# danyang-rainbow/trlx-t5

Measured on AMD Instinct MI355X. Metric: PPO experience+loss tokens/sec and % HBM roofline, 1/2/4/8 MI355X, higher is better.
Workload: dtype f32; 1 GPU; C2 GPT-2 sentiments PPO shape: 128 x 48 response tokens, vocab 50257, bf16 logits; rows_per_gpu=128, global_batch=128, seq_len=48, vocab=50257, logits_dtype=bf16, parallelism=dp1, schedule=pipelined

## Files before the change

include/trlx_t5_amd.h:

```cpp
#ifndef TRLX_T5_AMD_H
#define TRLX_T5_AMD_H

#include <stdint.h>

#ifdef __cplusplus
extern "C" {
#endif

#define TRLX_ABI_VERSION 2

typedef enum {
    TRLX_F32 = 0,
    TRLX_BF16 = 1,
    TRLX_I64 = 2,
} trlx_dtype;

typedef enum {
    TRLX_OK = 0,
    TRLX_ERR_SHAPE = 1,
    TRLX_ERR_STRIDE = 2,
    TRLX_ERR_DTYPE = 3,
    TRLX_ERR_LAUNCH = 4,
    TRLX_ERR_ARG = 5,
} trlx_status;
// ... 506 lines not shown
    float* rew_kl;
    float* rew_score;
    double* stats8;
    int mom_lag;
    void* workspace;
} trlx_gae_split_args;
int trlx_ppo_loss_rows_split_gae(const void* logits, int dtype, int64_t B, int64_t T, int64_t V, int64_t sb,
                                 int64_t st, const int64_t* labels, int64_t lb, int64_t lt, const void* old_lp,
                                 int old_dtype, const float* adv0, const float* adv_kl, const float* rew_kl,
                                 const float* rew_score, const double* stats8, int unbiased, const double* ctl_state,
                                 float kl_coef, float* coef, const double* msum, const int64_t* mask,
                                 const void* values, int v_dtype, const void* old_values, int ov_dtype,
                                 float* rewards, void* returns, int r_dtype, float cliprange, float cliprange_value,
                                 float vf_coef, float* lp_out, void* dx, int64_t dsb, int64_t dst, float* dvalues,
                                 void* workspace, const trlx_gae_split_args* gae, void* stream, void* done_event);

int trlx_comm_load(const char* librccl_path);
int64_t trlx_comm_unique_id_bytes(void);
int trlx_comm_unique_id(void* id_out, int64_t nbytes);
int trlx_comm_init(void** comm_out, const void* id, int64_t nbytes, int nranks, int rank);
int trlx_comm_allreduce_sum_f64(void* comm, double* buf, int64_t n, void* stream);
int trlx_comm_destroy(void* comm);

int trlx_scale_by(const void* x, void* out, int dtype, int64_t n, const float* scale, void* stream);

#ifdef __cplusplus
}
#endif
#endif
```

trlx-t5_amd/_lib.py:

```python
import contextlib
import ctypes
import os

import torch

_HERE = os.path.dirname(os.path.abspath(__file__))
LIB_PATH = os.environ.get("TRLX_T5_AMD_LIB") or os.path.join(_HERE, "libtrlx_t5_amd.so")

F32, BF16, I64 = 0, 1, 2
ABI_VERSION = 2
MOMENT_SLOTS = 4
SPLIT_MOMENT_SLOTS = 8
PPO_STATS = 13
PPO_PARTIAL_SLOTS = 16

_c_vp, _c_i64, _c_int, _c_f, _c_d = ctypes.c_void_p, ctypes.c_int64, ctypes.c_int, ctypes.c_float, ctypes.c_double


class IlqlArgs(ctypes.Structure):
    _fields_ = [
        ("dtype", _c_int), ("nq", _c_int),
        ("B", _c_i64), ("L", _c_i64), ("A", _c_i64), ("V", _c_i64),
        ("logits", _c_vp), ("logits_sb", _c_i64), ("logits_st", _c_i64),
        ("q", _c_vp * 2), ("q_sb", _c_i64 * 2), ("q_st", _c_i64 * 2),
# ... 236 lines not shown
    "trlx_ppo_rollout_loss_ctl": (_c_int, [_c_i64, _c_i64, _c_vp, _c_f, _c_vp, _c_vp, _c_vp, _kl_ctl_p, _c_vp]),
    "trlx_ppo_rollout_gae_split": (_c_int, [_c_i64, _c_i64, _c_vp, _c_vp, _c_vp, _c_int, _c_vp, _c_vp, _c_vp,
                                            _score_ctl_p, _c_f, _c_d, _c_d, _c_vp, _c_vp, _c_vp, _c_vp, _c_vp,
                                            _c_vp, _c_vp, _c_int, _c_int, _c_vp, _c_vp, _c_vp]),
    "trlx_score_moments_merge": (_c_int, [_c_vp, _c_vp, _c_vp, _c_vp]),
    "trlx_ppo_whiten_coef": (_c_int, [_c_vp, _c_int, _c_vp, _c_f, _c_vp, _c_vp]),
    "trlx_ppo_loss_rows_split": (_c_int, [_c_vp, _c_int, _c_i64, _c_i64, _c_i64, _c_i64, _c_i64, _c_vp, _c_i64,
                                          _c_i64, _c_vp, _c_int, _c_vp, _c_vp, _c_vp, _c_vp, _c_vp, _c_vp, _c_vp,
                                          _c_vp, _c_int, _c_vp, _c_int, _c_vp, _c_vp, _c_int, _c_f, _c_f, _c_f,
                                          _c_vp, _c_vp, _c_i64, _c_i64, _c_vp, _c_vp, _c_vp]),
    "trlx_ppo_loss_rows_split_gae": (_c_int, [_c_vp, _c_int, _c_i64, _c_i64, _c_i64, _c_i64, _c_i64, _c_vp, _c_i64,
                                              _c_i64, _c_vp, _c_int, _c_vp, _c_vp, _c_vp, _c_vp, _c_vp, _c_int, _c_vp,
                                              _c_f, _c_vp, _c_vp, _c_vp, _c_vp, _c_int, _c_vp, _c_int, _c_vp, _c_vp,
                                              _c_int, _c_f, _c_f, _c_f, _c_vp, _c_vp, _c_i64, _c_i64, _c_vp, _c_vp,
                                              _gae_split_p, _c_vp, _c_vp]),
    "trlx_comm_load": (_c_int, [ctypes.c_char_p]),
    "trlx_comm_unique_id_bytes": (_c_i64, []),
    "trlx_comm_unique_id": (_c_int, [_c_vp, _c_i64]),
    "trlx_comm_init": (_c_int, [ctypes.POINTER(ctypes.c_void_p), _c_vp, _c_i64, _c_int, _c_int]),
    "trlx_comm_allreduce_sum_f64": (_c_int, [_c_vp, _c_vp, _c_i64, _c_vp]),
    "trlx_comm_destroy": (_c_int, [_c_vp]),
    "trlx_lsm_gather_fwd_loss_tail": (_c_int, [_c_vp, _c_vp, _c_int, _c_i64, _c_i64, _c_i64, _c_i64, _c_i64, _c_vp,
                                               _c_i64, _c_i64, _c_vp, _c_vp, _c_vp, _c_vp, _c_int, _c_i64, _c_i64,
                                               _c_vp, _c_f, _c_vp, _c_vp, _c_vp, _kl_ctl_p, _c_vp]),
    "trlx_ilql_workspace_bytes": (_c_i64, [_c_i64, _c_i64, _c_i64, _c_int]),
    "trlx_ilql_prep": (_c_int, [_ilql_p, _c_vp]),
    "trlx_ilql_rows": (_c_int, [_ilql_p, _c_vp]),
    "trlx_ilql_finalize": (_c_int, [_ilql_p, _c_vp]),
    "trlx_ilql_loss_fused": (_c_int, [_ilql_p, _c_vp]),
    "trlx_ilql_tq_at_actions": (_c_int, [_ilql_tq_p, _c_vp]),
# ... 43 lines not shown
    _lib = lib
    return lib


def call(name, *args):
    lib = load()
    rc = getattr(lib, name)(*args)
    if rc != 0:
        msg = lib.trlx_last_error().decode(errors="replace")
        err = ValueError if rc in (1, 2, 3, 5) else TrlxError
        raise err(f"{name} failed (status {rc}): {msg}")
    return rc


_TUNED = {}


def set_tuning(key: str, value: int):
    call("trlx_set_tuning", key.encode(), int(value))
    _TUNED[key] = int(value)


@contextlib.contextmanager
def tuning(**knobs):
    prev = {k: _TUNED.get(k, 0) for k in knobs}
    try:
        for k, v in knobs.items():
            set_tuning(k, v)
        yield
    finally:
        for k, v in prev.items():
            set_tuning(k, v)


def query(name, *args):
    return getattr(load(), name)(*args)


def dtype_code(t):
    if t.dtype == torch.float32:
# ... 21 lines not shown
```

trlx-t5_amd/csrc/vocab_rows.hip:

```cpp
#include <string>

#include <hip/hip_ext.h>

#include "ppo_token.h"
#include "row_order.h"

namespace trlx {

enum RowMode { kFwd = 0, kBwd = 1, kPpo = 2 };

struct RowArgs {
    const void* x0;
    const void* x1;
    int64_t B, T, V, sb, st;
    const int64_t* labels;
    int64_t lb, lt;
    void* lp0;
    void* lp1;
    int out_dtype;
    float* lse0;
    float* lse1;
    const float* lse_in;
    const void* grad;
    int grad_dtype;
// ... 20 lines not shown
    int lead_blocks;
    void* done_event;
    const float* coef;
    const float* adv_kl;
    const float* rew_kl;
    const float* rew_score;
    float* rewards_out;
    const double* wstats;
    int wunbiased;
    const double* wctl;
    float wbeta;
    float* coef_out;
    const int64_t* lengths;
    const int* row_list;
    int* order_ws;
};

__global__ void k_whiten_coef(const double* stats, int unbiased, const double* ctl_state, float host_beta,
                              float* coef) {
    if (threadIdx.x == 0)
        whiten_coef_split(stats, unbiased, ctl_state ? float(ctl_state[TRLX_CTL_KL_COEF]) : host_beta, coef);
}

__global__ __launch_bounds__(kRolloutThreads) void k_rollout_loss(LossRolloutArgs L) {
    __shared__ double red[kRolloutsPerBlock * 16];
    loss_tail_block(L, int(blockIdx.x), int(gridDim.x), red);
}

template <class DT>
struct Row {
// ... 116 lines not shown

__device__ __forceinline__ bool any_masked(const RowArgs& a) {
    const double msum = a.msum ? *a.msum : a.msum_host;
    return msum != double(a.B * a.T);
}

template <class DT>
__device__ __forceinline__ void masked_row(const RowArgs& a, int64_t row) {
    typedef typename DT::elem_t E;
    const int64_t b = row / a.T, t = row - b * a.T;
    E* drow = reinterpret_cast<E*>(a.dx) + b * a.dsb + t * a.dst;
    const RowSplit<DT> s(drow, a.V);
    const int tid = threadIdx.x, nthr = blockDim.x;
    const __amdgpu_buffer_rsrc_t rout = make_rsrc(drow + s.head, uint32_t(s.nvec) * 16u);
    const vec4u z = {0u, 0u, 0u, 0u};
    for (int i = tid; i < int(s.nvec); i += nthr) store_grad_b128(z, rout, i * 16, a.spol);
    if (tid < s.head) DT::store1(drow, tid, 0.0f);
    if (tid < s.tail) DT::store1(drow, s.tail0 + tid, 0.0f);
    if (tid == 0) {
        float vin[3];
        const PpoScalars p = ppo_scalars(a, row, vin, true);
        PolicyTerms pt;
        ppo_policy_dlp(0.0f, p.olp, p.A, p.m, p.inv_msum, a.cliprange, pt);
        a.lp_out[row] = 0.0f;
        token_record(a, row, pt, p, vin);
        if (a.coef || a.wstats) split_outputs(a, row, p);
    }
}

template <class DT, int NV, int MODE, bool SAME_PHASE, bool LB512, int NL, int WPE, bool MASKED>
__device__ __forceinline__ void vocab_row(const RowArgs& a, int64_t row) {
    __shared__ float sh_max[kMaxThreads / kWave];
    __shared__ float sh_max2[kMaxThreads / kWave];
// ... 213 lines not shown
                    DT::unpack(lds_row[kk * 512 + tid], f);
#pragma unroll
                    for (int e = 0; e < EPV; ++e) {
                        const int64_t j = r.s.head + int64_t(i) * EPV + e;
                        DT::store1(drow, j, j == r.y ? gy : ng * exp2_fast(fmaf(f[e], kLog2e, lse_l2e)));
                    }
                }
            }
        }
    }
    if (MODE == kPpo && tid == 0) {
        const PolicyTerms t2 = {s_tok[0], s_tok[1], s_tok[2], s_tok[3] != 0.f};
        const PpoScalars p2 = {0.f, s_tok[4], s_tok[5], 0.f, s_ps[7], s_ps[8], s_ps[9], s_ps[10], s_ps[11]};
        token_record(a, r.row, t2, p2, s_ps + 4);
        if (a.coef || a.wstats) split_outputs(a, r.row, p2);
    }
}

template <class DT, int NV, int MODE, bool SAME_PHASE, bool LB512, int NL = 0, int WPE = 4, bool MASKED = false>
__global__ __launch_bounds__((LB512 || NL) ? 512 : kMaxThreads, LB512 ? 8 : (NL ? WPE : 1)) void k_vocab_rows(RowArgs a) {
    if constexpr (MODE == kFwd) {
        if (int(blockIdx.x) < a.tail_blocks) {
            __shared__ double tail_red[kMaxThreads / kWave * 16];
            if (blockIdx.y == 0) loss_tail_block(a.tail, int(blockIdx.x), a.tail_blocks, tail_red);
            return;
        }
    }
    if constexpr (MODE == kPpo && NL > 0) {
        if (int(blockIdx.x) < a.gae_blocks) {
            __shared__ double gae_red[kMaxThreads / kWave * 8];
// ... 147 lines not shown
                    DT::store1(drow, j, j == r.y ? gy : f[e]);
                }
            }
        }
    }
    if (je >= 0) DT::store1(drow, je, je == r.y ? gy : ng * exp2_fast(fmaf(ex, kLog2e, lse_l2e)));
    if (MODE == kPpo && a.tokrec && tid == 0) {
        PpoScalars p2 = ps;
        if (a.coef || a.wstats)
            split_value_inputs(a, r.row, split_advantage(a, r.row, ps.beta), vin, p2.R);
        else
            loss_token_inputs(a.ltok, r.row, vin);
        token_record(a, r.row, pt, ps, vin);
        if (a.coef || a.wstats) split_outputs(a, r.row, p2);
    }
}

struct Geometry {
    int nv;
    int threads;
};

static TuneKnob g_row_variant{0};
static TuneKnob g_resident_threads{0};
static TuneKnob g_resident_lb512{0};
static TuneKnob g_stream_threads{0};
static TuneKnob g_stream_unroll{0};
static TuneKnob g_row_order{0};
static TuneKnob g_ragged_order{0};
static TuneKnob g_order_launch{0};
static TuneKnob g_store_pol{0};
constexpr double kSC1Bytes = 1.5e9;

static int store_policy_for(double grad_bytes, bool split) {
    if (g_store_pol == 5) return kStoreNT;
    if (g_store_pol) return g_store_pol;
    return (!split && grad_bytes > kSC1Bytes) ? kStoreSC1 : kStoreNT;
}
static TuneKnob g_split_lds{0};
static TuneKnob g_split_mid{0};
int tuning_split_lds() { return g_split_lds; }
static TuneKnob g_ilql_split{0};
int tuning_ilql_split() { return g_ilql_split; }

static const int kNVs[] = {1, 2, 3, 4, 5, 6, 7, 8, 10, 12, 13, 16};

// ... 58 lines not shown

static int rows_grid(RowArgs& a, int threads, int nten, hipStream_t stream, dim3& grid, bool split) {
    const int rc = lead_standalone(a, stream, false, !split || threads < kRolloutThreads);
    if (rc) return rc;
    a.tail_blocks = a.has_tail ? int((a.tail.B + threads / kWave - 1) / (threads / kWave)) : 0;
    a.gae_blocks = a.has_gae ? int((a.gae.B + kRolloutsPerBlock - 1) / kRolloutsPerBlock) : 0;
    a.lead_blocks = a.tail_blocks + a.gae_blocks;
    grid = dim3(unsigned(a.B * a.T + a.lead_blocks), unsigned(nten));
    return TRLX_OK;
}

template <int MODE, class DT>
static int launch_rows_dt(const RowArgs& a0, int nten, hipStream_t stream) {
    RowArgs a = a0;
    a.order = g_row_order;
    const double grad_bytes = double(a.B) * double(a.T) * double(a.V) * double(sizeof(typename DT::elem_t));
    a.spol = MODE == kFwd ? kStoreNT : store_policy_for(grad_bytes, true);
    if constexpr (sizeof(typename DT::elem_t) == 2) {
        const int64_t nvec = a.V / 8 + 1 + (kLineVecs - 1);
        const bool want = g_split_lds == 2 || (g_split_lds == 0 && MODE != kFwd);
        if (want && !g_row_variant && !g_resident_threads && nvec > 512 * 8 && nvec <= 512 * (9 + 4)) {
            dim3 grid;
            const int rc = rows_grid(a, 512, nten, stream, grid, true);
            if (rc) return rc;
            if (MODE == kFwd || rows_same_phase(a, 2))
                TRLX_RESIDENT_LAUNCH(DT, 9, true, false, 4, 6, grid, dim3(512), stream, a);
            else
                TRLX_RESIDENT_LAUNCH(DT, 9, false, false, 4, 6, grid, dim3(512), stream, a);
            return check_launch("k_vocab_rows (split LDS, bf16)");
        }
// ... 335 lines not shown
                                         int64_t lb, int64_t lt, const void* values, int v_dtype,
                                         const float* scores, const int64_t* lengths, const int64_t* mask,
                                         float kl_coef, double gamma, double lam, float* lp, float* ref_lp,
                                         float* rewards, float* adv_raw, void* ret, int ret_dtype,
                                         double* stats, void* workspace, void* stream) {
    TRLX_REQUIRE(ref_logits && workspace, TRLX_ERR_ARG, "NULL reference logits / workspace");
    Workspace ws;
    carve_workspace(workspace, B, T, &ws);
    int rc = trlx_lsm_gather_fwd_ragged(logits, ref_logits, dtype, B, T, V, sb, st, labels, lb, lt, lengths, ws.order,
                                        lp, ref_lp, TRLX_F32, stream);
    if (rc) return rc;
    return trlx_ppo_rollout_gae(B, T, lp, ref_lp, values, v_dtype, scores, lengths, mask, kl_coef, gamma, lam,
                                rewards, adv_raw, ret, ret_dtype, stats, workspace, stream);
}

extern "C" int trlx_ppo_loss_rows(const void* logits, int dtype, int64_t B, int64_t T, int64_t V, int64_t sb,
                                  int64_t st, const int64_t* labels, int64_t lb, int64_t lt, const void* old_lp,
                                  int old_dtype, const float* adv_raw, const double* stats, int unbiased,
                                  const int64_t* mask, const void* values, int v_dtype, const void* old_values,
                                  int ov_dtype, const void* returns, int r_dtype, float cliprange,
                                  float cliprange_value, float vf_coef, float* lp_out, void* dx, int64_t dsb,
                                  int64_t dst, float* dvalues, void* workspace, void* stream) {
    RowArgs a = {};
    a.x0 = logits; a.B = B; a.T = T; a.V = V; a.sb = sb; a.st = st; a.labels = labels; a.lb = lb; a.lt = lt;
    a.old_lp = old_lp; a.old_dtype = old_dtype; a.adv = adv_raw; a.stats = stats; a.unbiased = unbiased;
    a.mask = mask; a.msum = stats ? stats + 3 : nullptr; a.msum_host = double(B * T); a.cliprange = cliprange;
    a.lp_out = lp_out; a.dx = dx; a.dsb = dsb; a.dst = dst;
    int rc = check_rows(a, dtype);
    if (rc) return rc;
    TRLX_REQUIRE(B > 0 && T > 0, TRLX_ERR_SHAPE, "empty rollout batch");
    TRLX_REQUIRE(old_lp && adv_raw && stats && values && old_values && returns && lp_out && dx && dvalues && workspace,
                 TRLX_ERR_ARG, "NULL argument to trlx_ppo_loss_rows");
    Workspace ws;
    carve_workspace(workspace, B, T, &ws);
    a.tokrec = ws.tokrec;
    a.ltok.values = values; a.ltok.v_dtype = v_dtype; a.ltok.old_values = old_values; a.ltok.ov_dtype = ov_dtype;
    a.ltok.returns = returns; a.ltok.r_dtype = r_dtype; a.ltok.cv = cliprange_value; a.ltok.vf_coef = vf_coef;
    a.ltok.dv = dvalues;
    return launch_rows<kPpo>(a, dtype, 1, (hipStream_t)stream);
}

extern "C" int trlx_ppo_loss_rows_split(const void* logits, int dtype, int64_t B, int64_t T, int64_t V, int64_t sb,
                                        int64_t st, const int64_t* labels, int64_t lb, int64_t lt, const void* old_lp,
                                        int old_dtype, const float* adv0, const float* adv_kl, const float* rew_kl,
                                        const float* rew_score, const float* coef, const double* msum,
                                        const int64_t* mask, const void* values, int v_dtype, const void* old_values,
                                        int ov_dtype, float* rewards, void* returns, int r_dtype, float cliprange,
                                        float cliprange_value, float vf_coef, float* lp_out, void* dx, int64_t dsb,
                                        int64_t dst, float* dvalues, void* workspace, void* stream) {
    RowArgs a = {};
    a.x0 = logits; a.B = B; a.T = T; a.V = V; a.sb = sb; a.st = st; a.labels = labels; a.lb = lb; a.lt = lt;
    a.old_lp = old_lp; a.old_dtype = old_dtype; a.adv = adv0; a.adv_kl = adv_kl; a.rew_kl = rew_kl;
    a.rew_score = rew_score; a.coef = coef; a.rewards_out = rewards;
    a.mask = mask; a.msum = msum; a.msum_host = double(B * T); a.cliprange = cliprange;
    a.lp_out = lp_out; a.dx = dx; a.dsb = dsb; a.dst = dst;
    int rc = check_rows(a, dtype);
    if (rc) return rc;
    TRLX_REQUIRE(B > 0 && T > 0, TRLX_ERR_SHAPE, "empty rollout batch");
    TRLX_REQUIRE(old_lp && adv0 && adv_kl && rew_kl && rew_score && coef && rewards && values && old_values &&
                 returns && lp_out && dx && dvalues && workspace, TRLX_ERR_ARG,
                 "NULL argument to trlx_ppo_loss_rows_split");
    TRLX_REQUIRE(r_dtype == TRLX_F32 || r_dtype == TRLX_BF16, TRLX_ERR_DTYPE, "returns dtype %d", r_dtype);
    Workspace ws;
    carve_workspace(workspace, B, T, &ws);
    a.tokrec = ws.tokrec;
    a.ltok.values = values; a.ltok.v_dtype = v_dtype; a.ltok.old_values = old_values; a.ltok.ov_dtype = ov_dtype;
    a.ltok.returns = returns; a.ltok.r_dtype = r_dtype; a.ltok.cv = cliprange_value; a.ltok.vf_coef = vf_coef;
    a.ltok.dv = dvalues;
    return launch_rows<kPpo>(a, dtype, 1, (hipStream_t)stream);
}

extern "C" int trlx_ppo_loss_rows_split_gae(
    const void* logits, int dtype, int64_t B, int64_t T, int64_t V, int64_t sb, int64_t st, const int64_t* labels,
    int64_t lb, int64_t lt, const void* old_lp, int old_dtype, const float* adv0, const float* adv_kl,
    const float* rew_kl, const float* rew_score, const double* stats8, int unbiased, const double* ctl_state,
    float kl_coef, float* coef, const double* msum, const int64_t* mask, const void* values, int v_dtype,
    const void* old_values, int ov_dtype, float* rewards, void* returns, int r_dtype, float cliprange,
    float cliprange_value, float vf_coef, float* lp_out, void* dx, int64_t dsb, int64_t dst, float* dvalues,
    void* workspace, const trlx_gae_split_args* gae, void* stream, void* done_event) {
    RowArgs a = {};
    a.x0 = logits; a.B = B; a.T = T; a.V = V; a.sb = sb; a.st = st; a.labels = labels; a.lb = lb; a.lt = lt;
    a.old_lp = old_lp; a.old_dtype = old_dtype; a.adv = adv0; a.adv_kl = adv_kl; a.rew_kl = rew_kl;
    a.rew_score = rew_score; a.rewards_out = rewards;
    a.wstats = stats8; a.wunbiased = unbiased; a.wctl = ctl_state; a.wbeta = kl_coef; a.coef_out = coef;
    a.mask = mask; a.msum = msum; a.msum_host = double(B * T); a.cliprange = cliprange;
    a.lp_out = lp_out; a.dx = dx; a.dsb = dsb; a.dst = dst;
    a.done_event = done_event;
    int rc = check_rows(a, dtype);
    if (rc) return rc;
    TRLX_REQUIRE(B > 0 && T > 0, TRLX_ERR_SHAPE, "empty rollout batch");
    TRLX_REQUIRE(old_lp && adv0 && adv_kl && rew_kl && rew_score && stats8 && rewards && values && old_values &&
                 returns && lp_out && dx && dvalues && workspace, TRLX_ERR_ARG,
                 "NULL argument to trlx_ppo_loss_rows_split_gae");
    TRLX_REQUIRE(r_dtype == TRLX_F32 || r_dtype == TRLX_BF16, TRLX_ERR_DTYPE, "returns dtype %d", r_dtype);
    Workspace ws;
    carve_workspace(workspace, B, T, &ws);
    a.tokrec = ws.tokrec;
    a.ltok.values = values; a.ltok.v_dtype = v_dtype; a.ltok.old_values = old_values; a.ltok.ov_dtype = ov_dtype;
    a.ltok.returns = returns; a.ltok.r_dtype = r_dtype; a.ltok.cv = cliprange_value; a.ltok.vf_coef = vf_coef;
    a.ltok.dv = dvalues;
    if (gae) {
// ... 2 lines not shown
                     (long long)gae->B, (long long)gae->T, (long long)B, (long long)T);
        TRLX_REQUIRE(gae->stats8 != stats8 && gae->adv0 != adv0 && gae->adv_kl != adv_kl, TRLX_ERR_ARG,
                     "the folded GAE must write the other split buffer set (it runs beside these rows)");
        const SplitGae sp = {gae->adv_kl, gae->rew_kl, gae->rew_score, nullptr, nullptr, 0, gae->mom_lag, nullptr};
        rc = fill_gae(a.gae, gae->B, gae->T, gae->lp, gae->ref_lp, gae->values, gae->v_dtype, gae->scores,
                      gae->lengths, gae->mask, gae->kl_coef, gae->ctl, gae->gamma, gae->lam, nullptr, gae->adv0,
                      nullptr, TRLX_F32, gae->stats8, gae->workspace, &sp);
        if (rc) return rc;
        TRLX_REQUIRE(!gae->ctl || (ctl_state != gae->ctl->state_out), TRLX_ERR_ARG,
                     "the rows read beta from the state the folded GAE writes (pass its state_in)");
        a.has_gae = 1;
    }
    return launch_rows<kPpo>(a, dtype, 1, (hipStream_t)stream);
}

static int fill_loss_tail(LossRolloutArgs* L, int64_t B, int64_t T, const double* stats, float vf_coef, float* loss,
                          float* loss_stats, void* workspace, const trlx_kl_ctl* kl) {
    TRLX_REQUIRE(B > 0 && T > 0, TRLX_ERR_SHAPE, "empty rollout batch");
    TRLX_REQUIRE(loss && loss_stats && workspace, TRLX_ERR_ARG, "NULL argument to the PPO loss tail");
    *L = {};
    carve_workspace(workspace, B, T, &L->ws);
    L->B = int(B); L->T = int(T); L->msum = stats ? stats + 3 : nullptr; L->vf_coef = vf_coef; L->loss = loss;
    L->stats = loss_stats;
    if (kl) {
        TRLX_REQUIRE(kl->state, TRLX_ERR_ARG, "trlx_kl_ctl.state is NULL");
        TRLX_REQUIRE(!kl->adaptive || (kl->target != 0.0 && kl->horizon != 0.0), TRLX_ERR_ARG,
                     "adaptive KL control needs target and horizon");
        L->kl.state = kl->state; L->kl.adaptive = kl->adaptive; L->kl.target = kl->target;
        L->kl.horizon = kl->horizon; L->kl.n_steps = double(kl->n_steps);
    }
// ... 45 lines not shown
                     "resident_threads must be a multiple of 64 <= %d", kMaxThreads);
        g_resident_threads = int(value);
    } else if (k == "stream_threads") {
        TRLX_REQUIRE(value == 0 || (value % kWave == 0 && value <= kStreamMaxThreads), TRLX_ERR_ARG,
                     "stream_threads must be a multiple of 64 <= %d", kStreamMaxThreads);
        g_stream_threads = int(value);
    } else if (k == "ilql_split") {
        TRLX_REQUIRE(value >= 0 && value <= 3, TRLX_ERR_ARG, "ilql_split: 0 (20+5), 1 (22+3), 2 (21+4), 3 (19+6)");
        g_ilql_split = int(value);
    } else if (k == "split_lds") {
        TRLX_REQUIRE(value >= 0 && value <= 2, TRLX_ERR_ARG, "split_lds: 0..2");
        g_split_lds = int(value);
    } else if (k == "store_policy") {
        TRLX_REQUIRE(value >= 0 && value <= 5, TRLX_ERR_ARG, "store_policy: 0..5");
        g_store_pol = int(value);
    } else if (k == "split_mid") {
        TRLX_REQUIRE(value >= 0 && value <= 3, TRLX_ERR_ARG, "split_mid: 0..3");
        g_split_mid = int(value);
    } else if (k == "order_launch") {
        TRLX_REQUIRE(value >= 0 && value <= 2, TRLX_ERR_ARG, "order_launch: 0 auto, 1 one launch, 2 two launches");
        g_order_launch = int(value);
    } else if (k == "ragged_order") {
        TRLX_REQUIRE(value == 0 || value == 1, TRLX_ERR_ARG, "ragged_order: 0 (valid rows first) or 1 (natural)");
        g_ragged_order = int(value);
    } else if (k == "row_order") {
        TRLX_REQUIRE(value == 0 || value == 1, TRLX_ERR_ARG, "row_order: 0 or 1");
        g_row_order = int(value);
    } else if (k == "stream_unroll") {
        TRLX_REQUIRE(value == 0 || value == 2 || value == 4 || value == 8, TRLX_ERR_ARG, "stream_unroll: 2, 4 or 8");
        g_stream_unroll = int(value);
// ... 12 lines not shown
```

trlx-t5_amd/lm_head.py:

```python
import ctypes

import torch

from . import _lib

__all__ = ["lm_head_logprobs", "PLANS"]

GRAD_HIDDEN_SIZES = (512, 768)


def _operands(hidden, weight, labels):
    H = hidden.shape[-1]
    h = hidden.reshape(-1, H)
    if h.stride(-1) != 1 or h.stride(0) % 8 or h.data_ptr() % 16:
        h = h.contiguous()
    w = weight if (weight.stride(-1) == 1 and weight.stride(0) % 8 == 0 and weight.data_ptr() % 16 == 0) \
        else weight.contiguous()
    return h, w, labels.reshape(-1).contiguous()


PLANS = ("auto", "saved_p", "recompute")


def _savep_buffer(N, H, V, dev, plan):
# ... 5 lines not shown
    try:
        return torch.empty(nbytes, dtype=torch.uint8, device=dev)
    except torch.cuda.OutOfMemoryError:
        return None


class _LmHeadLogprobs(torch.autograd.Function):

    @staticmethod
    def forward(ctx, hidden, weight, labels, out_dtype, plan, mask):
        h, w, y = _operands(hidden, weight, labels)
        N, H, V = h.shape[0], h.shape[1], w.shape[0]
        dev = h.device
        lp = torch.empty(N, dtype=out_dtype, device=dev)
        lse = torch.empty(N, dtype=torch.float32, device=dev)
        e = torch.empty((N, H), dtype=torch.float32, device=dev)
        saved = _savep_buffer(N, H, V, dev, plan) if ctx.needs_input_grad[1] else None
        ws = torch.empty(_lib.query("trlx_lmhead_loss_workspace_bytes", N, H, V), dtype=torch.uint8, device=dev)
        plan_token = ctypes.c_int64(0)
        _lib.call("trlx_lmhead_logprobs_fwd_ex2", h.data_ptr(), h.stride(0), w.data_ptr(), w.stride(0), N, H, V,
                  y.data_ptr(), 1, _lib.ptr(mask), lp.data_ptr(), _lib.dtype_code(lp), lse.data_ptr(), e.data_ptr(),
                  ws.data_ptr(), _lib.ptr(saved), ctypes.byref(plan_token), _lib.stream_of(h))
        del ws
        ctx.save_for_backward(h, w, y, lse, e, mask, saved)
        ctx.plan_token = plan_token.value
        ctx.shapes = (hidden.shape, hidden.dtype, weight.shape, weight.dtype)
        return lp.view(labels.shape)

    @staticmethod
    def backward(ctx, grad_lp):
        h, w, y, lse, e, mask, saved_p = ctx.saved_tensors
# ... 65 lines not shown
```

trlx-t5_amd/step.py:

```python
from typing import Optional

import ctypes

import torch
import torch.distributed as dist

from . import _lib
from .modeling import grad_buffer_like
from .control import PPOControlState
from .ppo import PPOConfig
from .comm import RcclComm
from .timing import LaunchEvent, make_event

__all__ = ["PPOHotPath"]


class _StreamJoin:

    __slots__ = ("_ev", "_dev", "_joined")

    def __init__(self, ev, device):
        self._ev, self._dev, self._joined = ev, device, None

    def wait(self):
# ... 58 lines not shown
        self.rewards = torch.empty((B, T), **f32)
        self.adv_raw = self._adv_raw4 = torch.empty((B, T), **f32)
        self.returns = torch.empty((B, T), dtype=value_dtype, device=self.device)
        self.lp_new = torch.empty((B, T), **f32)
        self.dvalues = torch.empty((B, T), **f32)
        self._stats4 = torch.empty(_lib.MOMENT_SLOTS, dtype=torch.float64, device=self.device)
        self.adv_stats = self._stats4
        self._split_mode = False
        self._coef_ready = False
        self._ar_msum = None
        self.loss = torch.empty(1, **f32)
        self.stats = torch.empty(_lib.PPO_STATS, **f32)
        nbytes = _lib.query("trlx_ppo_workspace_bytes", B, T)
        self.workspace = torch.zeros(nbytes, dtype=torch.uint8, device=self.device)
        self.dlogits = None
        self.lm_ws = None
        self.lm_logits = None
        self.lm_loss_ws = None
        self.distributed = False
        self._loss_ws_fallback = False
        self.timers = None
        self.timer_names = None
        self._conv = {}
        self._order_ws = None
        self._ar_work = None
        self._ar_group = None
        self._lp_bufs = None
        self._pending = None

    def _ev(self, name, s):
# ... 358 lines not shown
            return
        w.wait()
        if self.loss_norm == "global":
            world = self.comm.nranks if self.comm is not None else dist.get_world_size(self._ar_group)
            self._ar_msum.div_(world)

    def policy_loss(self, new_logits, labels, values, old_values, mask=None, _fold=None):
        self._check(new_logits)
        B, T, V = self.B, self.T, self.V
        labels = self._int64(labels, (B, T), "labels")
        mask = self._int64(mask, (B, T), "mask", required=False)
        values = self._vec(values, (B, T), "values")
        old_values = self._vec(old_values, (B, T), "old_values")
        if self.dlogits is None or self.dlogits.stride() != new_logits.stride():
            self.dlogits = grad_buffer_like(new_logits)
        s = torch.cuda.current_stream(self.device)
        self._launch_pending_tail(s)
        if self.tail_done is not None:
            self.tail_done.wait(s)
        dx = self.dlogits
        rows = (new_logits.data_ptr(), _lib.dtype_code(new_logits), B, T, V, new_logits.stride(0),
                new_logits.stride(1), labels.data_ptr(), labels.stride(0), labels.stride(1), self.lp_old.data_ptr(),
                _lib.F32)
        grads = (float(self.cfg.cliprange), float(self.cfg.cliprange_value), float(self.cfg.vf_coef),
                 self.lp_new.data_ptr(), dx.data_ptr(), dx.stride(0), dx.stride(1), self.dvalues.data_ptr(),
                 self.workspace.data_ptr())
        if _fold is not None and not (self._split_mode and not self._coef_ready):
            raise RuntimeError("a folded GAE rides the first split-beta loss launch of an experience")
        if self._split_mode:
            sb = self._sbuf[self._sidx]
            split = (sb["adv0"].data_ptr(), sb["adv_kl"].data_ptr(), sb["rew_kl"].data_ptr(),
                     sb["rew_score"].data_ptr())
            vals = (sb["stats"].data_ptr() + 6 * 8, _lib.ptr(mask), values.data_ptr(), _lib.dtype_code(values),
                    old_values.data_ptr(), _lib.dtype_code(old_values), self.rewards.data_ptr(),
                    self.returns.data_ptr(), _lib.dtype_code(self.returns))
            self._ev("loss", s)
            if not self._coef_ready and not self._derive_coef and _fold is None:
                _lib.call("trlx_ppo_whiten_coef", sb["stats"].data_ptr(), 0 if self.distributed else 1,
                          self.ctl.state.data_ptr() if self.ctl is not None else None, self.kl_coef,
                          sb["coef"].data_ptr(), s.cuda_stream)
                self._coef_ready = True
            if self._coef_ready:
                _lib.call("trlx_ppo_loss_rows_split", *rows, *split, sb["coef"].data_ptr(), *vals, *grads,
                          s.cuda_stream)
            else:
                if _fold is not None:
                    beta_state = _fold["beta_state"]
                else:
                    beta_state = self.ctl.state.data_ptr() if self.ctl is not None else None
                done = _fold["done"] if _fold is not None else None
                _lib.call("trlx_ppo_loss_rows_split_gae", *rows, *split, sb["stats"].data_ptr(),
                          0 if self.distributed else 1, beta_state, self.kl_coef, sb["coef"].data_ptr(), *vals,
                          *grads, ctypes.byref(_fold["args"]) if _fold is not None else None, s.cuda_stream,
                          done.handle if done is not None else None)
                self._coef_ready = True
            tail_stats = sb["stats"].data_ptr() + 3 * 8
        else:
            self._ev("loss", s)
            _lib.call("trlx_ppo_loss_rows", *rows, self.adv_raw.data_ptr(), self.adv_stats.data_ptr(),
                      0 if self.distributed else 1, _lib.ptr(mask), values.data_ptr(), _lib.dtype_code(values),
                      old_values.data_ptr(), _lib.dtype_code(old_values), self.returns.data_ptr(),
                      _lib.dtype_code(self.returns), *grads, s.cuda_stream)
            tail_stats = self.adv_stats.data_ptr()
        self._ev_end("loss", s)
        self._loss_tail(s, tail_stats)
        return self.loss, self.stats, self.dlogits, self.dvalues

    def _loss_tail(self, s, tail_stats):
        ts = s
        if self.tail_stream is not None:
            rows_done = self._next_event()
            rows_done.record(s)
            ts = self.tail_stream
            rows_done.wait(ts)
        args = (self.B, self.T, tail_stats, float(self.cfg.vf_coef), self.loss.data_ptr(), self.stats.data_ptr(),
                self.workspace.data_ptr())
        if self.defer_tail:
            self._tail_pending = args
            return
        self._ev("rollout_loss", ts)
        if self.ctl is not None:
# ... 277 lines not shown
```

Baseline: 15.91 million tokens/s.

## Track per-row dlogits dirty state to skip redundant zeroing of masked rows

Adds a per-row byte state for the gradient buffer. Masked rows whose dlogits are already zero skip the full-vocab zero store, and rows that get written mark themselves dirty. The Python side invalidates the state whenever the buffer pointer or version changes. This removes repeated zero writes over the large bf16 dlogits buffer across iterations, at the cost of extra state bookkeeping, a block barrier, and correctness that depends on nobody else modifying the buffer. The LM head also now zero-initialises its buffer when a mask is given.

```diff
diff --git a/include/trlx_t5_amd.h b/include/trlx_t5_amd.h
--- a/include/trlx_t5_amd.h
+++ b/include/trlx_t5_amd.h
@@ -544,6 +544,31 @@
                                  float* rewards, void* returns, int r_dtype, float cliprange, float cliprange_value,
                                  float vf_coef, float* lp_out, void* dx, int64_t dsb, int64_t dst, float* dvalues,
                                  void* workspace, const trlx_gae_split_args* gae, void* stream, void* done_event);
+int trlx_ppo_loss_rows_ex(const void* logits, int dtype, int64_t B, int64_t T, int64_t V, int64_t sb, int64_t st,
+                          const int64_t* labels, int64_t lb, int64_t lt, const void* old_lp, int old_dtype,
+                          const float* adv_raw, const double* stats, int unbiased, const int64_t* mask,
+                          const void* values, int v_dtype, const void* old_values, int ov_dtype,
+                          const void* returns, int r_dtype, float cliprange, float cliprange_value, float vf_coef,
+                          float* lp_out, void* dx, int64_t dsb, int64_t dst, uint8_t* dx_state, float* dvalues,
+                          void* workspace, void* stream);
+int trlx_ppo_loss_rows_split_ex(const void* logits, int dtype, int64_t B, int64_t T, int64_t V, int64_t sb,
+                                int64_t st, const int64_t* labels, int64_t lb, int64_t lt, const void* old_lp,
+                                int old_dtype, const float* adv0, const float* adv_kl, const float* rew_kl,
+                                const float* rew_score, const float* coef, const double* msum, const int64_t* mask,
+                                const void* values, int v_dtype, const void* old_values, int ov_dtype,
+                                float* rewards, void* returns, int r_dtype, float cliprange, float cliprange_value,
+                                float vf_coef, float* lp_out, void* dx, int64_t dsb, int64_t dst, uint8_t* dx_state,
+                                float* dvalues, void* workspace, void* stream);
+int trlx_ppo_loss_rows_split_gae_ex(const void* logits, int dtype, int64_t B, int64_t T, int64_t V, int64_t sb,
+                                    int64_t st, const int64_t* labels, int64_t lb, int64_t lt, const void* old_lp,
+                                    int old_dtype, const float* adv0, const float* adv_kl, const float* rew_kl,
+                                    const float* rew_score, const double* stats8, int unbiased,
+                                    const double* ctl_state, float kl_coef, float* coef, const double* msum,
+                                    const int64_t* mask, const void* values, int v_dtype, const void* old_values,
+                                    int ov_dtype, float* rewards, void* returns, int r_dtype, float cliprange,
+                                    float cliprange_value, float vf_coef, float* lp_out, void* dx, int64_t dsb,
+                                    int64_t dst, uint8_t* dx_state, float* dvalues, void* workspace,
+                                    const trlx_gae_split_args* gae, void* stream, void* done_event);
 
 int trlx_comm_load(const char* librccl_path);
 int64_t trlx_comm_unique_id_bytes(void);
diff --git a/trlx-t5_amd/_lib.py b/trlx-t5_amd/_lib.py
--- a/trlx-t5_amd/_lib.py
+++ b/trlx-t5_amd/_lib.py
@@ -274,6 +274,19 @@
                                               _c_f, _c_vp, _c_vp, _c_vp, _c_vp, _c_int, _c_vp, _c_int, _c_vp, _c_vp,
                                               _c_int, _c_f, _c_f, _c_f, _c_vp, _c_vp, _c_i64, _c_i64, _c_vp, _c_vp,
                                               _gae_split_p, _c_vp, _c_vp]),
+    "trlx_ppo_loss_rows_ex": (_c_int, [_c_vp, _c_int, _c_i64, _c_i64, _c_i64, _c_i64, _c_i64, _c_vp, _c_i64, _c_i64,
+                                       _c_vp, _c_int, _c_vp, _c_vp, _c_int, _c_vp, _c_vp, _c_int, _c_vp, _c_int,
+                                       _c_vp, _c_int, _c_f, _c_f, _c_f, _c_vp, _c_vp, _c_i64, _c_i64, _c_vp, _c_vp,
+                                       _c_vp, _c_vp]),
+    "trlx_ppo_loss_rows_split_ex": (_c_int, [_c_vp, _c_int, _c_i64, _c_i64, _c_i64, _c_i64, _c_i64, _c_vp, _c_i64,
+                                             _c_i64, _c_vp, _c_int, _c_vp, _c_vp, _c_vp, _c_vp, _c_vp, _c_vp, _c_vp,
+                                             _c_vp, _c_int, _c_vp, _c_int, _c_vp, _c_vp, _c_int, _c_f, _c_f, _c_f,
+                                             _c_vp, _c_vp, _c_i64, _c_i64, _c_vp, _c_vp, _c_vp, _c_vp]),
+    "trlx_ppo_loss_rows_split_gae_ex": (_c_int, [_c_vp, _c_int, _c_i64, _c_i64, _c_i64, _c_i64, _c_i64, _c_vp, _c_i64,
+                                                 _c_i64, _c_vp, _c_int, _c_vp, _c_vp, _c_vp, _c_vp, _c_vp, _c_int,
+                                                 _c_vp, _c_f, _c_vp, _c_vp, _c_vp, _c_vp, _c_int, _c_vp, _c_int, _c_vp,
+                                                 _c_vp, _c_int, _c_f, _c_f, _c_f, _c_vp, _c_vp, _c_i64, _c_i64, _c_vp,
+                                                 _c_vp, _c_vp, _gae_split_p, _c_vp, _c_vp]),
     "trlx_comm_load": (_c_int, [ctypes.c_char_p]),
     "trlx_comm_unique_id_bytes": (_c_i64, []),
     "trlx_comm_unique_id": (_c_int, [_c_vp, _c_i64]),
@@ -347,6 +360,7 @@
 
 
 _TUNED = {}
+_TUNE_DEFAULTS = {"dx_state": 1}
 
 
 def set_tuning(key: str, value: int):
@@ -356,7 +370,7 @@
 
 @contextlib.contextmanager
 def tuning(**knobs):
-    prev = {k: _TUNED.get(k, 0) for k in knobs}
+    prev = {k: _TUNED.get(k, _TUNE_DEFAULTS.get(k, 0)) for k in knobs}
     try:
         for k, v in knobs.items():
             set_tuning(k, v)
diff --git a/trlx-t5_amd/csrc/vocab_rows.hip b/trlx-t5_amd/csrc/vocab_rows.hip
--- a/trlx-t5_amd/csrc/vocab_rows.hip
+++ b/trlx-t5_amd/csrc/vocab_rows.hip
@@ -58,6 +58,7 @@
     const int64_t* lengths;
     const int* row_list;
     int* order_ws;
+    uint8_t* dx_state;
 };
 
 __global__ void k_whiten_coef(const double* stats, int unbiased, const double* ctl_state, float host_beta,
@@ -204,9 +205,16 @@
     const int tid = threadIdx.x, nthr = blockDim.x;
     const __amdgpu_buffer_rsrc_t rout = make_rsrc(drow + s.head, uint32_t(s.nvec) * 16u);
     const vec4u z = {0u, 0u, 0u, 0u};
-    for (int i = tid; i < int(s.nvec); i += nthr) store_grad_b128(z, rout, i * 16, a.spol);
-    if (tid < s.head) DT::store1(drow, tid, 0.0f);
-    if (tid < s.tail) DT::store1(drow, s.tail0 + tid, 0.0f);
+    const bool dirty = !a.dx_state || a.dx_state[row] != 0;
+    if (dirty) {
+        for (int i = tid; i < int(s.nvec); i += nthr) store_grad_b128(z, rout, i * 16, a.spol);
+        if (tid < s.head) DT::store1(drow, tid, 0.0f);
+        if (tid < s.tail) DT::store1(drow, s.tail0 + tid, 0.0f);
+    }
+    if (a.dx_state) {
+        __syncthreads();
+        if (tid == 0 && dirty) a.dx_state[row] = 0;
+    }
     if (tid == 0) {
         float vin[3];
         const PpoScalars p = ppo_scalars(a, row, vin, true);
@@ -450,6 +458,9 @@
         const PpoScalars p2 = {0.f, s_tok[4], s_tok[5], 0.f, s_ps[7], s_ps[8], s_ps[9], s_ps[10], s_ps[11]};
         token_record(a, r.row, t2, p2, s_ps + 4);
         if (a.coef || a.wstats) split_outputs(a, r.row, p2);
+        if constexpr (MASKED) {
+            if (a.dx_state) a.dx_state[r.row] = 1;
+        }
     }
 }
 
@@ -627,6 +638,7 @@
         token_record(a, r.row, pt, ps, vin);
         if (a.coef || a.wstats) split_outputs(a, r.row, p2);
     }
+    if (MODE == kPpo && tid == 0 && a.mask && a.dx_state) a.dx_state[r.row] = 1;
 }
 
 struct Geometry {
@@ -643,6 +655,7 @@
 static TuneKnob g_ragged_order{0};
 static TuneKnob g_order_launch{0};
 static TuneKnob g_store_pol{0};
+static TuneKnob g_dx_state{1};
 constexpr double kSC1Bytes = 1.5e9;
 
 static int store_policy_for(double grad_bytes, bool split) {
@@ -731,6 +744,7 @@
 static int launch_rows_dt(const RowArgs& a0, int nten, hipStream_t stream) {
     RowArgs a = a0;
     a.order = g_row_order;
+    if (!g_dx_state) a.dx_state = nullptr;
     const double grad_bytes = double(a.B) * double(a.T) * double(a.V) * double(sizeof(typename DT::elem_t));
     a.spol = MODE == kFwd ? kStoreNT : store_policy_for(grad_bytes, true);
     if constexpr (sizeof(typename DT::elem_t) == 2) {
@@ -1096,18 +1110,19 @@
                                 rewards, adv_raw, ret, ret_dtype, stats, workspace, stream);
 }
 
-extern "C" int trlx_ppo_loss_rows(const void* logits, int dtype, int64_t B, int64_t T, int64_t V, int64_t sb,
-                                  int64_t st, const int64_t* labels, int64_t lb, int64_t lt, const void* old_lp,
-                                  int old_dtype, const float* adv_raw, const double* stats, int unbiased,
-                                  const int64_t* mask, const void* values, int v_dtype, const void* old_values,
-                                  int ov_dtype, const void* returns, int r_dtype, float cliprange,
-                                  float cliprange_value, float vf_coef, float* lp_out, void* dx, int64_t dsb,
-                                  int64_t dst, float* dvalues, void* workspace, void* stream) {
+extern "C" int trlx_ppo_loss_rows_ex(const void* logits, int dtype, int64_t B, int64_t T, int64_t V, int64_t sb,
+                                     int64_t st, const int64_t* labels, int64_t lb, int64_t lt, const void* old_lp,
+                                     int old_dtype, const float* adv_raw, const double* stats, int unbiased,
+                                     const int64_t* mask, const void* values, int v_dtype, const void* old_values,
+                                     int ov_dtype, const void* returns, int r_dtype, float cliprange,
+                                     float cliprange_value, float vf_coef, float* lp_out, void* dx, int64_t dsb,
+                                     int64_t dst, uint8_t* dx_state, float* dvalues, void* workspace,
+                                     void* stream) {
     RowArgs a = {};
     a.x0 = logits; a.B = B; a.T = T; a.V = V; a.sb = sb; a.st = st; a.labels = labels; a.lb = lb; a.lt = lt;
     a.old_lp = old_lp; a.old_dtype = old_dtype; a.adv = adv_raw; a.stats = stats; a.unbiased = unbiased;
     a.mask = mask; a.msum = stats ? stats + 3 : nullptr; a.msum_host = double(B * T); a.cliprange = cliprange;
-    a.lp_out = lp_out; a.dx = dx; a.dsb = dsb; a.dst = dst;
+    a.lp_out = lp_out; a.dx = dx; a.dsb = dsb; a.dst = dst; a.dx_state = dx_state;
     int rc = check_rows(a, dtype);
     if (rc) return rc;
     TRLX_REQUIRE(B > 0 && T > 0, TRLX_ERR_SHAPE, "empty rollout batch");
@@ -1122,20 +1137,33 @@
     return launch_rows<kPpo>(a, dtype, 1, (hipStream_t)stream);
 }
 
-extern "C" int trlx_ppo_loss_rows_split(const void* logits, int dtype, int64_t B, int64_t T, int64_t V, int64_t sb,
-                                        int64_t st, const int64_t* labels, int64_t lb, int64_t lt, const void* old_lp,
-                                        int old_dtype, const float* adv0, const float* adv_kl, const float* rew_kl,
-                                        const float* rew_score, const float* coef, const double* msum,
-                                        const int64_t* mask, const void* values, int v_dtype, const void* old_values,
-                                        int ov_dtype, float* rewards, void* returns, int r_dtype, float cliprange,
-                                        float cliprange_value, float vf_coef, float* lp_out, void* dx, int64_t dsb,
-                                        int64_t dst, float* dvalues, void* workspace, void* stream) {
+extern "C" int trlx_ppo_loss_rows(const void* logits, int dtype, int64_t B, int64_t T, int64_t V, int64_t sb,
+                                  int64_t st, const int64_t* labels, int64_t lb, int64_t lt, const void* old_lp,
+                                  int old_dtype, const float* adv_raw, const double* stats, int unbiased,
+                                  const int64_t* mask, const void* values, int v_dtype, const void* old_values,
+                                  int ov_dtype, const void* returns, int r_dtype, float cliprange,
+                                  float cliprange_value, float vf_coef, float* lp_out, void* dx, int64_t dsb,
+                                  int64_t dst, float* dvalues, void* workspace, void* stream) {
+    return trlx_ppo_loss_rows_ex(logits, dtype, B, T, V, sb, st, labels, lb, lt, old_lp, old_dtype, adv_raw, stats,
+                                 unbiased, mask, values, v_dtype, old_values, ov_dtype, returns, r_dtype, cliprange,
+                                 cliprange_value, vf_coef, lp_out, dx, dsb, dst, nullptr, dvalues, workspace, stream);
+}
+
+extern "C" int trlx_ppo_loss_rows_split_ex(const void* logits, int dtype, int64_t B, int64_t T, int64_t V, int64_t sb,
+                                           int64_t st, const int64_t* labels, int64_t lb, int64_t lt,
+                                           const void* old_lp, int old_dtype, const float* adv0, const float* adv_kl,
+                                           const float* rew_kl, const float* rew_score, const float* coef,
+                                           const double* msum, const int64_t* mask, const void* values, int v_dtype,
+                                           const void* old_values, int ov_dtype, float* rewards, void* returns,
+                                           int r_dtype, float cliprange, float cliprange_value, float vf_coef,
+                                           float* lp_out, void* dx, int64_t dsb, int64_t dst, uint8_t* dx_state,
+                                           float* dvalues, void* workspace, void* stream) {
     RowArgs a = {};
     a.x0 = logits; a.B = B; a.T = T; a.V = V; a.sb = sb; a.st = st; a.labels = labels; a.lb = lb; a.lt = lt;
     a.old_lp = old_lp; a.old_dtype = old_dtype; a.adv = adv0; a.adv_kl = adv_kl; a.rew_kl = rew_kl;
     a.rew_score = rew_score; a.coef = coef; a.rewards_out = rewards;
     a.mask = mask; a.msum = msum; a.msum_host = double(B * T); a.cliprange = cliprange;
-    a.lp_out = lp_out; a.dx = dx; a.dsb = dsb; a.dst = dst;
+    a.lp_out = lp_out; a.dx = dx; a.dsb = dsb; a.dst = dst; a.dx_state = dx_state;
     int rc = check_rows(a, dtype);
     if (rc) return rc;
     TRLX_REQUIRE(B > 0 && T > 0, TRLX_ERR_SHAPE, "empty rollout batch");
@@ -1152,21 +1180,35 @@
     return launch_rows<kPpo>(a, dtype, 1, (hipStream_t)stream);
 }
 
-extern "C" int trlx_ppo_loss_rows_split_gae(
+extern "C" int trlx_ppo_loss_rows_split(const void* logits, int dtype, int64_t B, int64_t T, int64_t V, int64_t sb,
+                                        int64_t st, const int64_t* labels, int64_t lb, int64_t lt, const void* old_lp,
+                                        int old_dtype, const float* adv0, const float* adv_kl, const float* rew_kl,
+                                        const float* rew_score, const float* coef, const double* msum,
+                                        const int64_t* mask, const void* values, int v_dtype, const void* old_values,
+                                        int ov_dtype, float* rewards, void* returns, int r_dtype, float cliprange,
+                                        float cliprange_value, float vf_coef, float* lp_out, void* dx, int64_t dsb,
+                                        int64_t dst, float* dvalues, void* workspace, void* stream) {
+    return trlx_ppo_loss_rows_split_ex(logits, dtype, B, T, V, sb, st, labels, lb, lt, old_lp, old_dtype, adv0, adv_kl,
+                                       rew_kl, rew_score, coef, msum, mask, values, v_dtype, old_values, ov_dtype,
+                                       rewards, returns, r_dtype, cliprange, cliprange_value, vf_coef, lp_out, dx, dsb,
+                                       dst, nullptr, dvalues, workspace, stream);
+}
+
+extern "C" int trlx_ppo_loss_rows_split_gae_ex(
     const void* logits, int dtype, int64_t B, int64_t T, int64_t V, int64_t sb, int64_t st, const int64_t* labels,
     int64_t lb, int64_t lt, const void* old_lp, int old_dtype, const float* adv0, const float* adv_kl,
     const float* rew_kl, const float* rew_score, const double* stats8, int unbiased, const double* ctl_state,
     float kl_coef, float* coef, const double* msum, const int64_t* mask, const void* values, int v_dtype,
     const void* old_values, int ov_dtype, float* rewards, void* returns, int r_dtype, float cliprange,
-    float cliprange_value, float vf_coef, float* lp_out, void* dx, int64_t dsb, int64_t dst, float* dvalues,
-    void* workspace, const trlx_gae_split_args* gae, void* stream, void* done_event) {
+    float cliprange_value, float vf_coef, float* lp_out, void* dx, int64_t dsb, int64_t dst, uint8_t* dx_state,
+    float* dvalues, void* workspace, const trlx_gae_split_args* gae, void* stream, void* done_event) {
     RowArgs a = {};
     a.x0 = logits; a.B = B; a.T = T; a.V = V; a.sb = sb; a.st = st; a.labels = labels; a.lb = lb; a.lt = lt;
     a.old_lp = old_lp; a.old_dtype = old_dtype; a.adv = adv0; a.adv_kl = adv_kl; a.rew_kl = rew_kl;
     a.rew_score = rew_score; a.rewards_out = rewards;
     a.wstats = stats8; a.wunbiased = unbiased; a.wctl = ctl_state; a.wbeta = kl_coef; a.coef_out = coef;
     a.mask = mask; a.msum = msum; a.msum_host = double(B * T); a.cliprange = cliprange;
-    a.lp_out = lp_out; a.dx = dx; a.dsb = dsb; a.dst = dst;
+    a.lp_out = lp_out; a.dx = dx; a.dsb = dsb; a.dst = dst; a.dx_state = dx_state;
     a.done_event = done_event;
     int rc = check_rows(a, dtype);
     if (rc) return rc;
@@ -1199,6 +1241,21 @@
     return launch_rows<kPpo>(a, dtype, 1, (hipStream_t)stream);
 }
 
+extern "C" int trlx_ppo_loss_rows_split_gae(
+    const void* logits, int dtype, int64_t B, int64_t T, int64_t V, int64_t sb, int64_t st, const int64_t* labels,
+    int64_t lb, int64_t lt, const void* old_lp, int old_dtype, const float* adv0, const float* adv_kl,
+    const float* rew_kl, const float* rew_score, const double* stats8, int unbiased, const double* ctl_state,
+    float kl_coef, float* coef, const double* msum, const int64_t* mask, const void* values, int v_dtype,
+    const void* old_values, int ov_dtype, float* rewards, void* returns, int r_dtype, float cliprange,
+    float cliprange_value, float vf_coef, float* lp_out, void* dx, int64_t dsb, int64_t dst, float* dvalues,
+    void* workspace, const trlx_gae_split_args* gae, void* stream, void* done_event) {
+    return trlx_ppo_loss_rows_split_gae_ex(logits, dtype, B, T, V, sb, st, labels, lb, lt, old_lp, old_dtype, adv0,
+                                           adv_kl, rew_kl, rew_score, stats8, unbiased, ctl_state, kl_coef, coef, msum,
+                                           mask, values, v_dtype, old_values, ov_dtype, rewards, returns, r_dtype,
+                                           cliprange, cliprange_value, vf_coef, lp_out, dx, dsb, dst, nullptr, dvalues,
+                                           workspace, gae, stream, done_event);
+}
+
 static int fill_loss_tail(LossRolloutArgs* L, int64_t B, int64_t T, const double* stats, float vf_coef, float* loss,
                           float* loss_stats, void* workspace, const trlx_kl_ctl* kl) {
     TRLX_REQUIRE(B > 0 && T > 0, TRLX_ERR_SHAPE, "empty rollout batch");
@@ -1274,6 +1331,9 @@
     } else if (k == "store_policy") {
         TRLX_REQUIRE(value >= 0 && value <= 5, TRLX_ERR_ARG, "store_policy: 0..5");
         g_store_pol = int(value);
+    } else if (k == "dx_state") {
+        TRLX_REQUIRE(value == 0 || value == 1, TRLX_ERR_ARG, "dx_state: 1 (default) or 0 (ignore the caller's state)");
+        g_dx_state = int(value);
     } else if (k == "split_mid") {
         TRLX_REQUIRE(value >= 0 && value <= 3, TRLX_ERR_ARG, "split_mid: 0..3");
         g_split_mid = int(value);
diff --git a/trlx-t5_amd/lm_head.py b/trlx-t5_amd/lm_head.py
--- a/trlx-t5_amd/lm_head.py
+++ b/trlx-t5_amd/lm_head.py
@@ -43,7 +43,7 @@
         dev = h.device
         lp = torch.empty(N, dtype=out_dtype, device=dev)
         lse = torch.empty(N, dtype=torch.float32, device=dev)
-        e = torch.empty((N, H), dtype=torch.float32, device=dev)
+        e = (torch.empty if mask is None else torch.zeros)((N, H), dtype=torch.float32, device=dev)
         saved = _savep_buffer(N, H, V, dev, plan) if ctx.needs_input_grad[1] else None
         ws = torch.empty(_lib.query("trlx_lmhead_loss_workspace_bytes", N, H, V), dtype=torch.uint8, device=dev)
         plan_token = ctypes.c_int64(0)
diff --git a/trlx-t5_amd/step.py b/trlx-t5_amd/step.py
--- a/trlx-t5_amd/step.py
+++ b/trlx-t5_amd/step.py
@@ -96,6 +96,9 @@
         nbytes = _lib.query("trlx_ppo_workspace_bytes", B, T)
         self.workspace = torch.zeros(nbytes, dtype=torch.uint8, device=self.device)
         self.dlogits = None
+        self._dx_state = None
+        self._dx_seen = None
+        self._dx_unmasked = False
         self.lm_ws = None
         self.lm_logits = None
         self.lm_loss_ws = None
@@ -484,7 +487,9 @@
         old_values = self._vec(old_values, (B, T), "old_values")
         if self.dlogits is None or self.dlogits.stride() != new_logits.stride():
             self.dlogits = grad_buffer_like(new_logits)
+            self._dx_state = None
         s = torch.cuda.current_stream(self.device)
+        dx_state = self._dlogits_state(mask)
         self._launch_pending_tail(s)
         if self.tail_done is not None:
             self.tail_done.wait(s)
@@ -493,8 +498,8 @@
                 new_logits.stride(1), labels.data_ptr(), labels.stride(0), labels.stride(1), self.lp_old.data_ptr(),
                 _lib.F32)
         grads = (float(self.cfg.cliprange), float(self.cfg.cliprange_value), float(self.cfg.vf_coef),
-                 self.lp_new.data_ptr(), dx.data_ptr(), dx.stride(0), dx.stride(1), self.dvalues.data_ptr(),
-                 self.workspace.data_ptr())
+                 self.lp_new.data_ptr(), dx.data_ptr(), dx.stride(0), dx.stride(1), _lib.ptr(dx_state),
+                 self.dvalues.data_ptr(), self.workspace.data_ptr())
         if _fold is not None and not (self._split_mode and not self._coef_ready):
             raise RuntimeError("a folded GAE rides the first split-beta loss launch of an experience")
         if self._split_mode:
@@ -511,7 +516,7 @@
                           sb["coef"].data_ptr(), s.cuda_stream)
                 self._coef_ready = True
             if self._coef_ready:
-                _lib.call("trlx_ppo_loss_rows_split", *rows, *split, sb["coef"].data_ptr(), *vals, *grads,
+                _lib.call("trlx_ppo_loss_rows_split_ex", *rows, *split, sb["coef"].data_ptr(), *vals, *grads,
                           s.cuda_stream)
             else:
                 if _fold is not None:
@@ -519,7 +524,7 @@
                 else:
                     beta_state = self.ctl.state.data_ptr() if self.ctl is not None else None
                 done = _fold["done"] if _fold is not None else None
-                _lib.call("trlx_ppo_loss_rows_split_gae", *rows, *split, sb["stats"].data_ptr(),
+                _lib.call("trlx_ppo_loss_rows_split_gae_ex", *rows, *split, sb["stats"].data_ptr(),
                           0 if self.distributed else 1, beta_state, self.kl_coef, sb["coef"].data_ptr(), *vals,
                           *grads, ctypes.byref(_fold["args"]) if _fold is not None else None, s.cuda_stream,
                           done.handle if done is not None else None)
@@ -527,14 +532,30 @@
             tail_stats = sb["stats"].data_ptr() + 3 * 8
         else:
             self._ev("loss", s)
-            _lib.call("trlx_ppo_loss_rows", *rows, self.adv_raw.data_ptr(), self.adv_stats.data_ptr(),
+            _lib.call("trlx_ppo_loss_rows_ex", *rows, self.adv_raw.data_ptr(), self.adv_stats.data_ptr(),
                       0 if self.distributed else 1, _lib.ptr(mask), values.data_ptr(), _lib.dtype_code(values),
                       old_values.data_ptr(), _lib.dtype_code(old_values), self.returns.data_ptr(),
                       _lib.dtype_code(self.returns), *grads, s.cuda_stream)
             tail_stats = self.adv_stats.data_ptr()
         self._ev_end("loss", s)
+        self._dx_seen = (self.dlogits.data_ptr(), self.dlogits._version)
         self._loss_tail(s, tail_stats)
         return self.loss, self.stats, self.dlogits, self.dvalues
+
+    def _dlogits_state(self, mask):
+        if mask is None or not _lib._TUNED.get("dx_state", 1):
+            self._dx_unmasked = True
+            return None
+        if self._dx_state is None:
+            self._dx_state = torch.empty(self.B * self.T, dtype=torch.uint8, device=self.device)
+            self._dx_seen = None
+        if self._dx_unmasked or self._dx_seen != (self.dlogits.data_ptr(), self.dlogits._version):
+            self._dx_state.fill_(1)
+            self._dx_unmasked = False
+        return self._dx_state
+
+    def invalidate_dlogits_state(self):
+        self._dx_seen = None
 
     def _loss_tail(self, s, tail_stats):
         ts = s
```

Result: no change. 15.89 million tokens/s (-0.1%).
